# sudhirverma/distributed-ranges

Hardware: AMD Instinct MI355X
Metric: elements/s & % HBM roofline: reduce/scan/sort/SpMV at 1/2/4/8 MI355X (higher is better)
Workload: dtype f32

## Files before the change

### distributed-ranges_amd/include/dr/shp/merge_sort.hpp

```cpp
#pragma once

#include <hip/hip_runtime.h>

#include <algorithm>
#include <cstddef>
#include <cstdint>

namespace shp::detail::msort {

constexpr int kMsBlock = 256;
template <typename T> constexpr int ipt() {
  return sizeof(T) <= 4 ? 8 : sizeof(T) <= 8 ? 8 : sizeof(T) <= 16 ? 4 : sizeof(T) <= 32 ? 2 : 1;
}
template <typename T> constexpr int pad_every() { return ipt<T>() >= 4 ? ipt<T>() : 0; }
template <typename T> constexpr std::size_t padded(std::size_t e) {
  return pad_every<T>() ? e + e / pad_every<T>() : e;
}
#ifndef DR_SHP_MSORT_SORT_THREADS
#define DR_SHP_MSORT_SORT_THREADS 256
#endif
static_assert(DR_SHP_MSORT_SORT_THREADS >= kMsBlock && (DR_SHP_MSORT_SORT_THREADS & (DR_SHP_MSORT_SORT_THREADS - 1)) == 0,
              "DR_SHP_MSORT_SORT_THREADS must be a power of two and at least kMsBlock");
template <typename T> constexpr int sort_threads() {
  return padded<T>(std::size_t(DR_SHP_MSORT_SORT_THREADS) * ipt<T>()) * sizeof(T) <= 65536 ? DR_SHP_MSORT_SORT_THREADS
                                                                                         : kMsBlock;
}
template <typename T> constexpr std::size_t tile() { return std::size_t(kMsBlock) * ipt<T>(); }
template <typename T> constexpr std::size_t sort_tile() { return std::size_t(sort_threads<T>()) * ipt<T>(); }

template <typename I, typename PA, typename PB, typename Comp>
__host__ __device__ inline I merge_path(PA a, I na, PB b, I nb, I diag, Comp &comp) {
  I lo = diag > nb ? diag - nb : 0, hi = diag < na ? diag : na;
  while (lo < hi) {
    const I mid = (lo + hi) / 2;
    if (!comp(b[diag - 1 - mid], a[mid])) lo = mid + 1;
    else hi = mid;
  }
  return lo;
}

template <typename T> struct lds_view {
  T *s;
  int off;
  __device__ T &operator[](int i) const {
    const int j = off + i;
    return s[pad_every<T>() ? j + j / pad_every<T>() : j];
  }
  __device__ lds_view at(int o) const { return {s, off + o}; }
};

template <int N, typename T, typename Comp>
__device__ inline int serial_merge(lds_view<T> v, int ai, int aend, int bi, int bend, T (&y)[N], Comp &comp) {
  int cnt = 0;
#pragma unroll
  for (int k = 0; k < N; k++) {
    if (ai < aend || bi < bend) {
      const bool take_b = bi < bend && (ai >= aend || comp(v[bi], v[ai]));
      if (take_b) y[k] = v[bi++];
      else y[k] = v[ai++];
      cnt = k + 1;
    }
  }
  return cnt;
}

template <typename T, std::size_t E> struct lds_tile {
  alignas(alignof(T) > 16 ? alignof(T) : 16) unsigned char raw[padded<T>(E) * sizeof(T)];
  __device__ lds_view<T> view() { return {reinterpret_cast<T *>(raw), 0}; }
};

template <typename T, typename Comp>
__global__ __launch_bounds__(sort_threads<T>()) void block_sort_kernel(T *data, std::size_t n, Comp comp) {
  constexpr int NT = sort_threads<T>();
  constexpr int N = ipt<T>();
  constexpr int TILE = (int)sort_tile<T>();
  __shared__ lds_tile<T, sort_tile<T>()> lds;
  const lds_view<T> s = lds.view();
  const std::size_t base = (std::size_t)blockIdx.x * TILE;
  const int cnt = (int)std::min<std::size_t>(TILE, n - base);
  {
    T r[N];
#pragma unroll
    for (int k = 0; k < N; k++)
      if (k * NT + (int)threadIdx.x < cnt) r[k] = data[base + k * NT + threadIdx.x];
#pragma unroll
    for (int k = 0; k < N; k++)
      if (k * NT + (int)threadIdx.x < cnt) s[k * NT + threadIdx.x] = r[k];
  }
  __syncthreads();
  const int my = threadIdx.x * N;
  const int valid = std::max(0, std::min(N, cnt - my));
  T x[N];
#pragma unroll
  for (int k = 0; k < N; k++)
    if (k < valid) x[k] = s[my + k];
#pragma unroll
  for (int r = 0; r < N; r++) {
#pragma unroll
    for (int k = r & 1; k + 1 < N; k += 2)
      if (k + 1 < valid && comp(x[k + 1], x[k])) {
        const T t = x[k];
        x[k] = x[k + 1];
        x[k + 1] = t;
      }
  }
  __syncthreads();
#pragma unroll
  for (int k = 0; k < N; k++)
    if (k < valid) s[my + k] = x[k];
  __syncthreads();
  for (int coop = 2; coop <= NT; coop *= 2) {
    const int lane = threadIdx.x % coop;
    const int g0 = (threadIdx.x / coop) * coop * N, half = coop / 2 * N;
    const int a0 = std::min(g0, cnt), a1 = std::min(g0 + half, cnt), b1 = std::min(g0 + 2 * half, cnt);
    const int na = a1 - a0, nb = b1 - a1;
    const int diag = std::min(lane * N, na + nb);
    const int i = merge_path<int>(s.at(a0), na, s.at(a1), nb, diag, comp);
    T y[N];
    const int got = serial_merge<N>(s, a0 + i, a1, a1 + diag - i, b1, y, comp);
    __syncthreads();
#pragma unroll
    for (int k = 0; k < N; k++)
      if (k < got) s[a0 + diag + k] = y[k];
    __syncthreads();
  }
#pragma unroll
  for (int k = 0; k < N; k++)
    if (k * NT + (int)threadIdx.x < cnt) data[base + k * NT + threadIdx.x] = s[k * NT + threadIdx.x];
}

struct pass_geom {
  std::size_t n, w;
  bool single;
  __host__ __device__ std::size_t pair_base(std::size_t d) const { return single ? 0 : d / (2 * w) * (2 * w); }
  __host__ __device__ std::size_t pair_end(std::size_t pb) const { return single ? n : std::min(n, pb + 2 * w); }
  __host__ __device__ std::size_t na(std::size_t pb) const { return std::min(w, n - pb); }
};

template <typename T, typename Comp>
__global__ void merge_partition_kernel(const T *src, pass_geom g, std::size_t ntiles, std::size_t *part, Comp comp) {
  const std::size_t t = (std::size_t)blockIdx.x * blockDim.x + threadIdx.x;
  if (t >= ntiles) return;
  const std::size_t d = t * tile<T>();
  const std::size_t pb = g.pair_base(d), na = g.na(pb), nb = g.pair_end(pb) - pb - na;
  part[t] = merge_path<std::size_t>(src + pb, na, src + pb + na, nb, d - pb, comp);
}

template <typename T, typename Comp>
__global__ __launch_bounds__(kMsBlock) void merge_kernel(const T *src, T *dst, pass_geom g, std::size_t ntiles,
                                                         const std::size_t *part, Comp comp) {
  constexpr int N = ipt<T>();
  constexpr std::size_t TILE = tile<T>();
  __shared__ lds_tile<T, tile<T>()> lds;
  const lds_view<T> s = lds.view();
  const std::size_t t = blockIdx.x;
  const std::size_t d0 = t * TILE, pb = g.pair_base(d0), pe = g.pair_end(pb);
  const std::size_t d1 = std::min(d0 + TILE, pe);
  const std::size_t na = g.na(pb);
  const std::size_t i0 = part[t];
  const std::size_t i1 = (t + 1 < ntiles && (t + 1) * TILE < pe) ? part[t + 1] : na;
  const std::size_t j0 = (d0 - pb) - i0, j1 = (d1 - pb) - i1;
  const T *A = src + pb, *B = src + pb + na;
  const int la = (int)(i1 - i0), lb = (int)(j1 - j0);
  {
    T r[N];
#pragma unroll
    for (int k = 0; k < N; k++) {
      const int e = k * kMsBlock + threadIdx.x;
      if (e < la) r[k] = A[i0 + e];
      else if (e < la + lb) r[k] = B[j0 + (e - la)];
    }
#pragma unroll
    for (int k = 0; k < N; k++) {
      const int e = k * kMsBlock + threadIdx.x;
      if (e < la + lb) s[e] = r[k];
    }
  }
  __syncthreads();
  const int diag = std::min((int)threadIdx.x * N, la + lb);
  const int i = merge_path<int>(s, la, s.at(la), lb, diag, comp);
  T y[N];
  const int got = serial_merge<N>(s, i, la, la + diag - i, la + lb, y, comp);
  __syncthreads();
#pragma unroll
  for (int k = 0; k < N; k++)
    if (k < got) s[diag + k] = y[k];
  __syncthreads();
#pragma unroll
  for (int k = 0; k < N; k++)
    if (k * kMsBlock + (int)threadIdx.x < la + lb) dst[d0 + k * kMsBlock + threadIdx.x] = s[k * kMsBlock + threadIdx.x];
}

template <typename T> __global__ void gather_samples_kernel(const T *data, std::size_t stride, std::size_t ns, T *s) {
  const std::size_t j = (std::size_t)blockIdx.x * blockDim.x + threadIdx.x;
  if (j < ns) s[j] = data[j * stride];
}

template <typename T> constexpr std::size_t scratch_bytes(std::size_t n) {
  const std::size_t tiles = (n + tile<T>() - 1) / tile<T>();
  return ((n * sizeof(T) + 255) & ~std::size_t(255)) + (tiles + 1) * sizeof(std::size_t);
}

inline unsigned blocks_of(std::size_t n, std::size_t per) { return (unsigned)std::max<std::size_t>(1, (n + per - 1) / per); }

template <typename T, typename Comp>
void merge_pass(const T *src, T *dst, pass_geom g, std::size_t *part, Comp comp, hipStream_t st) {
  const std::size_t ntiles = (g.n + tile<T>() - 1) / tile<T>();
  hipLaunchKernelGGL((merge_partition_kernel<T, Comp>), dim3(blocks_of(ntiles, 256)), dim3(256), 0, st, src, g,
                     ntiles, part, comp);
  hipLaunchKernelGGL((merge_kernel<T, Comp>), dim3((unsigned)ntiles), dim3(kMsBlock), 0, st, src, dst, g, ntiles,
                     part, comp);
}

template <typename T, typename Comp>
void local_sort(T *data, std::size_t n, void *scratch, Comp comp, hipStream_t st) {
  if (n <= 1) return;
  T *tmp = static_cast<T *>(scratch);
  auto *part = reinterpret_cast<std::size_t *>(static_cast<char *>(scratch) + ((n * sizeof(T) + 255) & ~std::size_t(255)));
  hipLaunchKernelGGL((block_sort_kernel<T, Comp>), dim3(blocks_of(n, sort_tile<T>())), dim3(sort_threads<T>()), 0,
                     st, data, n, comp);
  T *src = data, *dst = tmp;
  for (std::size_t w = sort_tile<T>(); w < n; w *= 2) {
    merge_pass<T>(src, dst, pass_geom{n, w, false}, part, comp, st);
    std::swap(src, dst);
  }
  if (src != data) (void)hipMemcpyAsync(data, src, n * sizeof(T), hipMemcpyDeviceToDevice, st);
}

}
```

Measured before the change: 541.9 billion.

## Choose ping-pong parity to skip final copy and widen merge tiles

The block sort now writes into whichever buffer makes the last merge pass land in the caller's array. This removes the trailing device-to-device memcpy when the pass count is odd. Merge kernels also use 16 items per thread for types up to 8 bytes, doubling the merge tile. That halves the partition count and blocks, at the cost of more registers and LDS per block and possibly lower occupancy.

Result: no change. 542.0 billion, median of 3 (+0.0%).

```diff
diff --git a/distributed-ranges_amd/include/dr/shp/merge_sort.hpp b/distributed-ranges_amd/include/dr/shp/merge_sort.hpp
--- a/distributed-ranges_amd/include/dr/shp/merge_sort.hpp
+++ b/distributed-ranges_amd/include/dr/shp/merge_sort.hpp
@@ -12,20 +12,20 @@
 template <typename T> constexpr int ipt() {
   return sizeof(T) <= 4 ? 8 : sizeof(T) <= 8 ? 8 : sizeof(T) <= 16 ? 4 : sizeof(T) <= 32 ? 2 : 1;
 }
-template <typename T> constexpr int pad_every() { return ipt<T>() >= 4 ? ipt<T>() : 0; }
-template <typename T> constexpr std::size_t padded(std::size_t e) {
-  return pad_every<T>() ? e + e / pad_every<T>() : e;
-}
+template <typename T> constexpr int merge_ipt() { return sizeof(T) <= 8 ? 16 : ipt<T>(); }
+template <int N> constexpr int pad_every() { return N >= 4 ? N : 0; }
+template <int N> constexpr std::size_t padded(std::size_t e) { return pad_every<N>() ? e + e / pad_every<N>() : e; }
 #ifndef DR_SHP_MSORT_SORT_THREADS
 #define DR_SHP_MSORT_SORT_THREADS 256
 #endif
 static_assert(DR_SHP_MSORT_SORT_THREADS >= kMsBlock && (DR_SHP_MSORT_SORT_THREADS & (DR_SHP_MSORT_SORT_THREADS - 1)) == 0,
               "DR_SHP_MSORT_SORT_THREADS must be a power of two and at least kMsBlock");
 template <typename T> constexpr int sort_threads() {
-  return padded<T>(std::size_t(DR_SHP_MSORT_SORT_THREADS) * ipt<T>()) * sizeof(T) <= 65536 ? DR_SHP_MSORT_SORT_THREADS
-                                                                                         : kMsBlock;
-}
-template <typename T> constexpr std::size_t tile() { return std::size_t(kMsBlock) * ipt<T>(); }
+  return padded<ipt<T>()>(std::size_t(DR_SHP_MSORT_SORT_THREADS) * ipt<T>()) * sizeof(T) <= 65536
+             ? DR_SHP_MSORT_SORT_THREADS
+             : kMsBlock;
+}
+template <typename T> constexpr std::size_t merge_tile() { return std::size_t(kMsBlock) * merge_ipt<T>(); }
 template <typename T> constexpr std::size_t sort_tile() { return std::size_t(sort_threads<T>()) * ipt<T>(); }
 
 template <typename I, typename PA, typename PB, typename Comp>
@@ -39,18 +39,18 @@
   return lo;
 }
 
-template <typename T> struct lds_view {
+template <typename T, int N> struct lds_view {
   T *s;
   int off;
   __device__ T &operator[](int i) const {
     const int j = off + i;
-    return s[pad_every<T>() ? j + j / pad_every<T>() : j];
+    return s[pad_every<N>() ? j + j / pad_every<N>() : j];
   }
   __device__ lds_view at(int o) const { return {s, off + o}; }
 };
 
 template <int N, typename T, typename Comp>
-__device__ inline int serial_merge(lds_view<T> v, int ai, int aend, int bi, int bend, T (&y)[N], Comp &comp) {
+__device__ inline int serial_merge(lds_view<T, N> v, int ai, int aend, int bi, int bend, T (&y)[N], Comp &comp) {
   int cnt = 0;
 #pragma unroll
   for (int k = 0; k < N; k++) {
@@ -64,25 +64,25 @@
   return cnt;
 }
 
-template <typename T, std::size_t E> struct lds_tile {
-  alignas(alignof(T) > 16 ? alignof(T) : 16) unsigned char raw[padded<T>(E) * sizeof(T)];
-  __device__ lds_view<T> view() { return {reinterpret_cast<T *>(raw), 0}; }
+template <typename T, int N, std::size_t E> struct lds_tile {
+  alignas(alignof(T) > 16 ? alignof(T) : 16) unsigned char raw[padded<N>(E) * sizeof(T)];
+  __device__ lds_view<T, N> view() { return {reinterpret_cast<T *>(raw), 0}; }
 };
 
 template <typename T, typename Comp>
-__global__ __launch_bounds__(sort_threads<T>()) void block_sort_kernel(T *data, std::size_t n, Comp comp) {
+__global__ __launch_bounds__(sort_threads<T>()) void block_sort_kernel(const T *src, T *dst, std::size_t n, Comp comp) {
   constexpr int NT = sort_threads<T>();
   constexpr int N = ipt<T>();
   constexpr int TILE = (int)sort_tile<T>();
-  __shared__ lds_tile<T, sort_tile<T>()> lds;
-  const lds_view<T> s = lds.view();
+  __shared__ lds_tile<T, N, sort_tile<T>()> lds;
+  const lds_view<T, N> s = lds.view();
   const std::size_t base = (std::size_t)blockIdx.x * TILE;
   const int cnt = (int)std::min<std::size_t>(TILE, n - base);
   {
     T r[N];
 #pragma unroll
     for (int k = 0; k < N; k++)
-      if (k * NT + (int)threadIdx.x < cnt) r[k] = data[base + k * NT + threadIdx.x];
+      if (k * NT + (int)threadIdx.x < cnt) r[k] = src[base + k * NT + threadIdx.x];
 #pragma unroll
     for (int k = 0; k < N; k++)
       if (k * NT + (int)threadIdx.x < cnt) s[k * NT + threadIdx.x] = r[k];
@@ -126,7 +126,7 @@
   }
 #pragma unroll
   for (int k = 0; k < N; k++)
-    if (k * NT + (int)threadIdx.x < cnt) data[base + k * NT + threadIdx.x] = s[k * NT + threadIdx.x];
+    if (k * NT + (int)threadIdx.x < cnt) dst[base + k * NT + threadIdx.x] = s[k * NT + threadIdx.x];
 }
 
 struct pass_geom {
@@ -141,7 +141,7 @@
 __global__ void merge_partition_kernel(const T *src, pass_geom g, std::size_t ntiles, std::size_t *part, Comp comp) {
   const std::size_t t = (std::size_t)blockIdx.x * blockDim.x + threadIdx.x;
   if (t >= ntiles) return;
-  const std::size_t d = t * tile<T>();
+  const std::size_t d = t * merge_tile<T>();
   const std::size_t pb = g.pair_base(d), na = g.na(pb), nb = g.pair_end(pb) - pb - na;
   part[t] = merge_path<std::size_t>(src + pb, na, src + pb + na, nb, d - pb, comp);
 }
@@ -149,10 +149,10 @@
 template <typename T, typename Comp>
 __global__ __launch_bounds__(kMsBlock) void merge_kernel(const T *src, T *dst, pass_geom g, std::size_t ntiles,
                                                          const std::size_t *part, Comp comp) {
-  constexpr int N = ipt<T>();
-  constexpr std::size_t TILE = tile<T>();
-  __shared__ lds_tile<T, tile<T>()> lds;
-  const lds_view<T> s = lds.view();
+  constexpr int N = merge_ipt<T>();
+  constexpr std::size_t TILE = merge_tile<T>();
+  __shared__ lds_tile<T, N, TILE> lds;
+  const lds_view<T, N> s = lds.view();
   const std::size_t t = blockIdx.x;
   const std::size_t d0 = t * TILE, pb = g.pair_base(d0), pe = g.pair_end(pb);
   const std::size_t d1 = std::min(d0 + TILE, pe);
@@ -197,7 +197,7 @@
 }
 
 template <typename T> constexpr std::size_t scratch_bytes(std::size_t n) {
-  const std::size_t tiles = (n + tile<T>() - 1) / tile<T>();
+  const std::size_t tiles = (n + merge_tile<T>() - 1) / merge_tile<T>();
   return ((n * sizeof(T) + 255) & ~std::size_t(255)) + (tiles + 1) * sizeof(std::size_t);
 }
 
@@ -205,26 +205,33 @@
 
 template <typename T, typename Comp>
 void merge_pass(const T *src, T *dst, pass_geom g, std::size_t *part, Comp comp, hipStream_t st) {
-  const std::size_t ntiles = (g.n + tile<T>() - 1) / tile<T>();
+  const std::size_t ntiles = (g.n + merge_tile<T>() - 1) / merge_tile<T>();
   hipLaunchKernelGGL((merge_partition_kernel<T, Comp>), dim3(blocks_of(ntiles, 256)), dim3(256), 0, st, src, g,
                      ntiles, part, comp);
   hipLaunchKernelGGL((merge_kernel<T, Comp>), dim3((unsigned)ntiles), dim3(kMsBlock), 0, st, src, dst, g, ntiles,
                      part, comp);
 }
 
+template <typename T> constexpr int merge_passes(std::size_t n) {
+  int r = 0;
+  for (std::size_t w = sort_tile<T>(); w < n; w *= 2) r++;
+  return r;
+}
+
 template <typename T, typename Comp>
 void local_sort(T *data, std::size_t n, void *scratch, Comp comp, hipStream_t st) {
+  static_assert((2 * sort_tile<T>()) % merge_tile<T>() == 0,
+                "a pair of block-sorted runs must be a whole number of merge tiles");
   if (n <= 1) return;
   T *tmp = static_cast<T *>(scratch);
   auto *part = reinterpret_cast<std::size_t *>(static_cast<char *>(scratch) + ((n * sizeof(T) + 255) & ~std::size_t(255)));
+  T *src = merge_passes<T>(n) % 2 ? tmp : data, *dst = src == data ? tmp : data;
   hipLaunchKernelGGL((block_sort_kernel<T, Comp>), dim3(blocks_of(n, sort_tile<T>())), dim3(sort_threads<T>()), 0,
-                     st, data, n, comp);
-  T *src = data, *dst = tmp;
+                     st, static_cast<const T *>(data), src, n, comp);
   for (std::size_t w = sort_tile<T>(); w < n; w *= 2) {
     merge_pass<T>(src, dst, pass_geom{n, w, false}, part, comp, st);
     std::swap(src, dst);
   }
-  if (src != data) (void)hipMemcpyAsync(data, src, n * sizeof(T), hipMemcpyDeviceToDevice, st);
-}
-
-}
+}
+
+}
```
